# catniplab/vjf

Hardware: AMD Instinct MI355X
Metric: trial-timesteps/sec (higher is better)
Workload: dtype f32

## Files before the change

### include/vjf_hip.h

```cpp
#ifndef VJF_HIP_H
#define VJF_HIP_H

#include <stdint.h>

#ifdef __cplusplus
extern "C" {
#endif

#define VJF_ABI_VERSION 1
#define VJF_MAX_HIDDEN 8

#define VJF_LIK_GAUSSIAN 0
#define VJF_LIK_POISSON 1

#define VJF_FLAG_SGD 1u
#define VJF_FLAG_UPDATE 2u
#define VJF_FLAG_WARM_UP 4u
#define VJF_FLAG_EXACT_NONFINITE 8u

#define VJF_STATUS_NONFINITE_RECON 1u
#define VJF_STATUS_NONFINITE_DYN 2u
#define VJF_STATUS_NONFINITE_ENT 4u
#define VJF_STATUS_RLS_FAILED 8u
#define VJF_STATUS_WAIT_RESIDENT 0x100u
// ... 40 lines not shown
    VJF_SC_FREEZE_DEC = 6,
    VJF_SC_STATUS = 7,
    VJF_SC_TRI_CLEAN = 8,
    VJF_SC_SHRINK = 9,
    VJF_N_SCALARS = 16
};

typedef struct vjf_config {
    int32_t ydim, xdim, udim, n_rbf;
    int32_t n_hidden;
    int32_t hidden[VJF_MAX_HIDDEN];
    int32_t likelihood;
    int32_t max_batch;
    int32_t device;
} vjf_config;

#define VJF_ACT_TANH 0
#define VJF_ACT_RELU 1
#define VJF_ACT_LEAKY_RELU 2
#define VJF_ACT_ELU 3
#define VJF_ACT_SOFTPLUS 4
#define VJF_ACT_SIGMOID 5
#define VJF_ACT_HARDTANH 6
typedef struct vjf_activation { int32_t kind; float p0, p1; } vjf_activation;

typedef struct vjf_ctx vjf_ctx;

int vjf_abi_version(void);
const char* vjf_last_error(void);

int vjf_state_size(const vjf_config* cfg, int64_t* n_floats);
int vjf_state_layout(const vjf_config* cfg, int64_t* offsets, int64_t* sizes);
int vjf_workspace_size(const vjf_config* cfg, int64_t* bytes);

int vjf_ctx_create(const vjf_config* cfg, float* state, void* workspace, int64_t workspace_bytes,
                   void* stream, vjf_ctx** out);
int vjf_ctx_destroy(vjf_ctx* ctx);
int vjf_set_activation(vjf_ctx* ctx, const vjf_activation* act);
int vjf_set_stream(vjf_ctx* ctx, void* stream);
int vjf_get_status(vjf_ctx* ctx, uint32_t* status);

int vjf_set_overlap(vjf_ctx* ctx, int enable);

int vjf_route(vjf_ctx* ctx, uint32_t flags);

int vjf_comm_unique_id(void* ids256);
int vjf_comm_init(vjf_ctx* ctx, const void* ids256, int32_t rank, int32_t world);
int vjf_set_collectives(vjf_ctx* ctx, int32_t per_step);
int vjf_comm_ranks(vjf_ctx* ctx, int32_t* ranks2);

int vjf_debug_stamps(vjf_ctx* ctx, int enable, uint64_t* out32);

int vjf_filter_step(vjf_ctx* ctx, int32_t B, const float* y, const float* u, const float* mu_s,
                    const float* lv_s, const float* eps_s, const float* eps_t, float* mu_t, float* lv_t,
                    float* loss4, uint32_t flags);

int vjf_filter_local(vjf_ctx* ctx, int32_t B, const float* y, const float* u, const float* mu_s,
                     const float* lv_s, const float* eps_s, const float* eps_t, float* mu_t, float* lv_t,
                     uint32_t flags);
int vjf_reduce_buffer(vjf_ctx* ctx, float** ptr, int64_t* n_floats);
int vjf_filter_global(vjf_ctx* ctx, int32_t B_total, float* loss4, uint32_t flags);

int vjf_filter_seq(vjf_ctx* ctx, int32_t T, int32_t B, const float* y, const float* u, const float* eps,
                   const float* mu0, const float* lv0, float* mu, float* lv, float* loss, uint32_t flags);

int vjf_rbf_forward(const float* x, const float* centroid, const float* logwidth, float* out,
// ... 77 lines not shown
```

### vjf_amd/_native.py

```python
import ctypes as C
import os

HERE = os.path.dirname(os.path.abspath(__file__))
_variant = os.environ.get("VJF_LIB", "")
LIB_PATH = os.path.join(HERE, f"libvjf_hip_{_variant}.so" if _variant.isalnum() else "libvjf_hip.so")

ABI_VERSION = 1
MAX_HIDDEN = 8
LIK_GAUSSIAN, LIK_POISSON = 0, 1
FLAG_SGD, FLAG_UPDATE, FLAG_WARM_UP, FLAG_EXACT_NONFINITE = 1, 2, 4, 8
STATUS_NONFINITE_RECON, STATUS_NONFINITE_DYN, STATUS_NONFINITE_ENT, STATUS_RLS_FAILED = 1, 2, 4, 8
STATUS_NOT_RESIDENT, STATUS_WAIT_MASK = 0x20000, 0x3ff00

SLOT_PRIOR_MEAN, SLOT_PRIOR_LOGVAR, SLOT_LIK_LOGVAR, SLOT_TR_LOGVAR, SLOT_CENTROID, SLOT_LOGWIDTH = range(6)
SLOT_REC_W0, SLOT_REC_B0 = 6, 7
SLOT_MEAN_W, SLOT_LV_W, SLOT_LV_B, SLOT_DEC_W, SLOT_DEC_B = 22, 23, 24, 25, 26
SLOT_W_MEAN, SLOT_W_CHOL, SLOT_W_PREC, SLOT_W_PCHOL, SLOT_SCALARS = 27, 28, 29, 30, 31
N_SLOTS = 32
SC_N_LIK, SC_N_TR, SC_LR_LIK, SC_LR_DEC, SC_LR_TR, SC_LR_REC, SC_FREEZE_DEC, SC_STATUS, SC_TRI_CLEAN, SC_SHRINK = range(10)
N_SCALARS = 16


ACT_TANH, ACT_RELU, ACT_LEAKY_RELU, ACT_ELU, ACT_SOFTPLUS, ACT_SIGMOID, ACT_HARDTANH = range(7)


class VjfActivation(C.Structure):
    _fields_ = [("kind", C.c_int32), ("p0", C.c_float), ("p1", C.c_float)]


class VjfError(RuntimeError):
    """A C-ABI call returned an error code."""


class VjfConfig(C.Structure):
    _fields_ = [("ydim", C.c_int32), ("xdim", C.c_int32), ("udim", C.c_int32), ("n_rbf", C.c_int32),
                ("n_hidden", C.c_int32), ("hidden", C.c_int32 * MAX_HIDDEN), ("likelihood", C.c_int32),
                ("max_batch", C.c_int32), ("device", C.c_int32)]


_P = C.c_void_p
_I = C.c_int32
_U = C.c_uint32
_F = C.c_float

SIGNATURES = {
    "vjf_abi_version": [],
    "vjf_state_size": [C.POINTER(VjfConfig), C.POINTER(C.c_int64)],
    "vjf_state_layout": [C.POINTER(VjfConfig), C.POINTER(C.c_int64), C.POINTER(C.c_int64)],
    "vjf_workspace_size": [C.POINTER(VjfConfig), C.POINTER(C.c_int64)],
    "vjf_ctx_create": [C.POINTER(VjfConfig), _P, _P, C.c_int64, _P, C.POINTER(_P)],
    "vjf_ctx_destroy": [_P],
    "vjf_set_activation": [_P, C.POINTER(VjfActivation)],
    "vjf_set_stream": [_P, _P],
    "vjf_get_status": [_P, C.POINTER(_U)],
    "vjf_set_overlap": [_P, _I],
    "vjf_route": [_P, _U],
    "vjf_comm_unique_id": [_P],
    "vjf_comm_init": [_P, _P, _I, _I],
    "vjf_comm_ranks": [_P, C.POINTER(_I)],
    "vjf_set_collectives": [_P, _I],
    "vjf_debug_stamps": [_P, _I, C.POINTER(C.c_uint64)],
    "vjf_filter_step": [_P, _I, _P, _P, _P, _P, _P, _P, _P, _P, _P, _U],
    "vjf_filter_local": [_P, _I, _P, _P, _P, _P, _P, _P, _P, _P, _U],
    "vjf_reduce_buffer": [_P, C.POINTER(_P), C.POINTER(C.c_int64)],
    "vjf_filter_global": [_P, _I, _P, _U],
    "vjf_filter_seq": [_P, _I, _I, _P, _P, _P, _P, _P, _P, _P, _P, _U],
    "vjf_rbf_forward": [_P, _P, _P, _P, _I, _I, _I, _P],
    "vjf_blr_predict": [_P, _P, _P, _P, _P, _P, _P, _I, _I, _I, _I, _P],
    "vjf_blr_sample": [_P, _P, _P, _P, _P, _P, _P, _P, _I, _I, _I, _I, _P],
    "vjf_forecast_scratch_size": [_I, _I, _I, C.POINTER(C.c_int64)],
    "vjf_forecast_seq": [_P, _P, _P, _P, _P, _P, _P, _P, _P, _P, _P, _I, _I, _I, _I, _I, _P],
    "vjf_forecast_ens_scratch_size": [_I, _I, _I, _I, _I, C.POINTER(C.c_int64)],
    "vjf_forecast_ens_chunks": [_I, _I, _I, _I, _I, C.POINTER(_I), C.POINTER(_I)],
    "vjf_forecast_ens": [_P, C.c_int64] + [_P] * 16 + [_I] * 7 + [_P],
    "vjf_tangent_plan": [_I, _I, _I, _I, C.POINTER(_I), C.POINTER(C.c_int64)],
    "vjf_tangent_rollout": [_P] * 10 + [_I] * 8 + [_P],
    "vjf_fixed_points_plan": [_I, _I, _I, C.POINTER(C.c_int64)],
    "vjf_fixed_points": [_P] * 10 + [_I] * 5 + [_F, _F, _P],
    "vjf_smooth_plan": [_I, _I, _I, C.POINTER(C.c_int64)],
    "vjf_smooth": [_P] * 12 + [_I] * 5 + [_F, _P],
    "vjf_smooth_sample_plan": [_I, _I, _I, _I, C.POINTER(_I), C.POINTER(C.c_int64)],
    "vjf_smooth_sample": [_P] * 9 + [_I] * 6 + [_F, _P],
# ... 84 lines not shown
```

### vjf_amd/csrc/vjf_abi.hip

```cpp
#include <hip/hip_runtime.h>
#include <hip/hip_ext.h>

#include <dlfcn.h>

#include <cstdarg>
#include <cstdio>
#include <cstdlib>
#include <cstring>
#include <ctime>
#include <atomic>
#include <mutex>
#include <new>
#include <string>
#include <type_traits>
#include <vector>

#include "../../include/vjf_hip.h"
#include "vjf_chol_blocks.h"
#include "vjf_chol_kernel.h"
#include "vjf_gram_kernel.h"
#include "vjf_handoff.h"
#include "vjf_mega_kernel.h"
#include "vjf_ops_kernels.h"
#include "vjf_plan.h"
// ... 31 lines not shown
#else
#define VJF_CHAOS_REFRESH(c) ((void)0)
#endif

extern "C" {

int vjf_abi_version(void) { return VJF_ABI_VERSION; }
const char* vjf_last_error(void) { return g_err.c_str(); }

int vjf_state_size(const vjf_config* cfg, int64_t* n_floats) {
    VjfPlan P;
    if (int rc = plan_for("vjf_state_size", cfg, &P)) return rc;
    if (!n_floats) return fail(-1, "vjf_state_size: null output");
    *n_floats = P.n_state;
    return 0;
}

int vjf_state_layout(const vjf_config* cfg, int64_t* offsets, int64_t* sizes) {
    VjfPlan P;
    if (int rc = plan_for("vjf_state_layout", cfg, &P)) return rc;
    if (!offsets || !sizes) return fail(-1, "vjf_state_layout: null output");
    for (int s = 0; s < VJF_N_SLOTS; ++s) { offsets[s] = P.off[s]; sizes[s] = P.size[s]; }
    return 0;
}

int vjf_workspace_size(const vjf_config* cfg, int64_t* bytes) {
    VjfPlan P;
    if (int rc = plan_for("vjf_workspace_size", cfg, &P)) return rc;
    if (!bytes) return fail(-1, "vjf_workspace_size: null output");
    if (cfg->max_batch < 1) return fail(-7, "vjf_workspace_size: max_batch must be >= 1");
    std::vector<VjfJob> jobs;
    build_jobs(P, jobs);
    *bytes = (int64_t)carve_ws(P, cfg->max_batch, (int)jobs.size()).total;
    return 0;
}

int vjf_ctx_create(const vjf_config* cfg, float* state, void* workspace, int64_t workspace_bytes, void* stream,
                   vjf_ctx** out) {
    if (!cfg || !state || !workspace || !out) return fail(-1, "vjf_ctx_create: null argument");
    VjfPlan P;
    if (int rc = plan_for("vjf_ctx_create", cfg, &P)) return rc;
    if (cfg->max_batch < 1) return fail(-7, "vjf_ctx_create: max_batch must be >= 1");
    std::vector<VjfJob> jobs;
    build_jobs(P, jobs);
    if ((int)jobs.size() > VJF_MAX_JOBS) return fail(-8, "vjf_ctx_create: %zu Gram tiles exceed the limit", jobs.size());
    Carve cv = carve_ws(P, cfg->max_batch, (int)jobs.size());
    if ((int64_t)cv.total > workspace_bytes)
        return fail(-9, "vjf_ctx_create: workspace too small (%lld < %zu bytes)", (long long)workspace_bytes, cv.total);
    const size_t lds_k2 = vjf_serial_lds_floats(P) * 4;
    const bool fast_chol = vjf_chol_lds_ok(P);
    if (!fast_chol && lds_k2 > kMaxLds - 1024 && P.n <= 32 * VJF_CHOL_MAXBLK)
        return fail(-11, "vjf_ctx_create: n_rbf=%d too large for the single-workgroup RLS kernel", P.n);
    VJF_HIP(hipSetDevice(cfg->device));
    vjf_ctx* c = new (std::nothrow) vjf_ctx();
    if (!c) return fail(-12, "vjf_ctx_create: out of host memory");
    c->cfg = *cfg; c->plan = P; c->state = state; c->ws = (char*)workspace; c->ws_bytes = workspace_bytes;
    c->stream = (hipStream_t)stream; c->cv = cv; c->njobs = (int)jobs.size();
    c->lds_k2 = lds_k2;
    c->fast_chol = fast_chol;
    c->lds_post = vjf_post_lds_bytes(P);
    c->post_kernels = fast_chol && P.dz <= 16 && c->lds_post <= kMaxLds - 1024;
    c->lds_chol = fast_chol ? kMaxLds - 256 : vjf_chol_lds_bytes(P);
    if (c->post_kernels) c->lds_post = kMaxLds - 256;
    c->lds_k1m = vjf_trial_mfma_lds_floats(P) * 4;
    c->mfma_trial = c->lds_k1m <= kMaxLds - 1024;
    for (const VjfJob& j : jobs) c->n_ejobs += j.kind == 0;
    { const char* ha = getenv("VJF_HANDOFF_ACQUIRE"); c->handoff_acquire = ha && atoi(ha) != 0; }
    c->mega_ok = c->mega_plan = mega_plan_ok(P);
    VJF_HIP(hipDeviceGetAttribute(&c->ncu, hipDeviceAttributeMultiprocessorCount, cfg->device));
    if (const char* ce = getenv("VJF_COLLECTIVES")) { if (atoi(ce) == 1) c->collectives = 1; }
    hipError_t e = hipMemcpyAsync(c->jobs(), jobs.data(), jobs.size() * sizeof(VjfJob), hipMemcpyHostToDevice, c->stream);
    if (e == hipSuccess) e = hipMemsetAsync(c->red(), 0, (size_t)P.red_len * 4, c->stream);
    if (e == hipSuccess) e = hipMemsetAsync(c->red_rls(0), 0, (size_t)P.red_len * 4, c->stream);
    if (e == hipSuccess) e = hipMemsetAsync(c->red_rls(1), 0, (size_t)P.red_len * 4, c->stream);
    if (e == hipSuccess) e = hipMemsetAsync(c->flag_words(), 0, 256, c->stream);
    SlabTables tb;
    if (c->mega_ok) {
        const VjfMegaTrialLds Lo = vjf_mega_trial_lds(P, (int)(kMegaLds / 4) - 8);
        tb = slab_tables(P, Lo, vjf_mega_slab_layout(P));
        if (e == hipSuccess) e = hipMemcpyAsync(c->mg_pidx(), tb.pidx.data(), tb.pidx.size() * 4, hipMemcpyHostToDevice, c->stream);
        if (e == hipSuccess) e = hipMemcpyAsync(c->mg_cidx(), tb.cidx.data(), tb.cidx.size() * 4, hipMemcpyHostToDevice, c->stream);
        if (e == hipSuccess) e = hipMemcpyAsync(c->mg_grp(), tb.grp.data(), tb.grp.size() * 4, hipMemcpyHostToDevice, c->stream);
        if (e == hipSuccess) e = hipMemsetAsync(c->mg_img(), 0, (size_t)Lo.th_len * 4, c->stream);
        if (e == hipSuccess) e = hipMemsetAsync(c->mega_counters(0), 0, (size_t)2 * MG_C_WORDS * 4, c->stream);
    }
    if (e == hipSuccess) e = hipStreamSynchronize(c->stream);
    if (e != hipSuccess) { delete c; return fail(-100, "vjf_ctx_create: %s", hipGetErrorString(e)); }
    allow_lds(vjf_serial_kernel, c->lds_k2);
    allow_lds(vjf_rls_post_kernel, c->lds_post);
    allow_lds(vjf_prepg_kernel, vjf_prepg_lds_bytes(P));
    if (c->mfma_trial) allow_lds(vjf_trial_mfma_kernel<>, c->lds_k1m);
    allow_lds(chol_kernels(P.dz).chol, c->lds_chol);
    if (P.dz <= 16) allow_lds(chol_kernels(P.dz).pair, c->lds_chol);
    mega_residency(c);
    if (DevShared* d = dev_shared(cfg->device)) {
        std::lock_guard<std::mutex> lk(d->mu);
        if (!d->mirror_h) {
            unsigned* h = nullptr; unsigned* dp = nullptr;
            if (hipHostMalloc((void**)&h, VJF_MIRROR_WORDS * sizeof(unsigned), hipHostMallocMapped | hipHostMallocCoherent) == hipSuccess &&
                hipHostGetDevicePointer((void**)&dp, h, 0) == hipSuccess) {
                memset(h, 0, VJF_MIRROR_WORDS * sizeof(unsigned));
                d->mirror_h = h; d->mirror_d = dp;
            }
            (void)hipGetLastError();
        }
        count_mega(c, d);
    }
    *out = c;
    return 0;
}

int vjf_ctx_destroy(vjf_ctx* ctx) {
    if (!ctx) return 0;
    if (DevShared* d = dev_shared(ctx->cfg.device)) {
        std::lock_guard<std::mutex> lk(d->mu);
// ... 592 lines not shown
```

### vjf_amd/csrc/vjf_host_ctx.h

```cpp
#pragma once

namespace {

thread_local std::string g_err;

int fail(int code, const char* fmt, ...) {
    char buf[512];
    va_list ap;
    va_start(ap, fmt);
    vsnprintf(buf, sizeof buf, fmt, ap);
    va_end(ap);
    g_err = buf;
    return code;
}

#define VJF_HIP(call)                                                                            \
    do {                                                                                         \
        hipError_t e_ = (call);                                                                  \
        if (e_ != hipSuccess) return fail(-100, "%s failed: %s (%s:%d)", #call, hipGetErrorString(e_), __FILE__, __LINE__); \
    } while (0)

#define VJF_LAUNCH(kernel, grid, block, lds, st, stop, ...)                                             \
    do {                                                                                               \
        if (stop) hipExtLaunchKernelGGL(kernel, grid, block, (uint32_t)(lds), st, nullptr, stop, 0, __VA_ARGS__); \
// ... 216 lines not shown
struct Carve {
    size_t pscr; size_t mg_mom, mg_xt, mg_early, mg_late, mg_gslab, mg_cnt, mg_stamps, mg_pidx, mg_cidx, mg_grp, mg_img, mg_pmsave; size_t E, E2, ACT, DEL, partial, partial2, slabs, red, red2, red3, tbig, wide, work, jobs, aux, post, lscr, flags, resid, total;
};

Carve carve_ws(const VjfPlan& P, int max_batch, int njobs) {
    Carve c{};
    size_t o = 0;
    auto take = [&](size_t bytes) { size_t at = o; o = (o + bytes + 255) / 256 * 256; return at; };
    c.E = take((size_t)max_batch * P.ldE * 4);
    c.E2 = take((size_t)max_batch * P.ldE * 4);
    c.ACT = take((size_t)max_batch * P.ldA * 4);
    c.DEL = take((size_t)max_batch * P.ldD * 4);
    c.partial = take(((size_t)max_batch / 4 + 2) * RS_N * 4);
    c.partial2 = take(((size_t)max_batch / 4 + 2) * RS_N * 4);
    c.slabs = take((size_t)njobs * split_for(max_batch) * 1024 * 4);
    c.red = take((size_t)P.red_len * 4);
    c.red2 = take((size_t)P.red_len * 4);
    c.red3 = take((size_t)P.red_len * 4);
    c.tbig = take(P.n > 32 * VJF_CHOL_MAXBLK ? (size_t)((P.n + 31) / 32) * 1024 * 4 * 3 : 16);
    c.wide = take(vjf_trial_mfma_lds_floats(P) * 4 > kMaxLds - 1024 ? (size_t)max_batch * (P.dxu + P.dz + 1 + P.dy + P.n) * 4 + 1024 : 16);
    c.work = take(vjf_serial_work_floats(P) * 4 + 10 * 256);
    c.post = take((size_t)((P.n + 31) / 32) * 1024 * 4 + VJF_RESID_BLOCKS * 8 + 64);
    c.flags = take(256);
    c.lscr = take((size_t)P.n * P.n * 4);
    c.pscr = take((size_t)(VJF_CHOL_MAXBLK * (VJF_CHOL_MAXBLK + 1) / 2) * 1024 * 4);
    if (mega_plan_ok(P)) {
        const int nbl = (P.n + 31) / 32;
        const size_t slab_len = (size_t)vjf_mega_slab_layout(P).len;
        c.mg_early = take((size_t)2 * kMegaMaxTrialWg * ((size_t)((P.n + 3) & ~3) * 16 + 8) * 4);
        c.mg_late = take((size_t)kMegaMaxTrialWg * (slab_len + 8 * VJF_MG_RING) * 4);
        c.mg_gslab = take((size_t)kMegaMaxGramWg * (nbl * (nbl + 1) / 2) * 1024 * 4);
        c.mg_cnt = take((size_t)2 * MG_C_WORDS * 4);
        c.mg_stamps = take((32 * 32 + kMegaMaxTrialWg * 8) * 8);
        c.mg_pidx = take(slab_len * 4); c.mg_cidx = take(slab_len * 4); c.mg_grp = take(slab_len);
        c.mg_img = take((size_t)vjf_mega_trial_lds(P, (int)(kMegaLds / 4) - 8).th_len * 4 + 64);
        c.mg_pmsave = take((size_t)max_batch * (P.dz + 1) * 4);
        c.mg_xt = take((size_t)P.n * P.n * 4);
        {
            int nt = (max_batch + VJF_MG_TR - 1) / VJF_MG_TR;
            if (nt > VJF_MG_TAG_TILES) nt = VJF_MG_TAG_TILES;
            c.mg_mom = take((size_t)nt * 2 * (2 * P.dz + 1) * VJF_MG_TR * 4);
        }
    }
    c.jobs = take((size_t)njobs * sizeof(VjfJob));
    c.aux = take((size_t)P.aux_len * 4);
    c.resid = take(P.n > 32 * VJF_CHOL_MAXBLK ? (size_t)max_batch * P.dz * 4 : 16);
    c.total = o;
    return c;
}

template <class K>
void allow_lds(K kernel, size_t bytes) {
    (void)hipFuncSetAttribute(reinterpret_cast<const void*>(kernel), hipFuncAttributeMaxDynamicSharedMemorySize, (int)bytes);
    (void)hipGetLastError();
}

}

struct vjf_ctx {
    vjf_config cfg{};
    VjfPlan plan{};
    float* state = nullptr;
    char* ws = nullptr;
    int64_t ws_bytes = 0;
    hipStream_t stream = nullptr;
    Carve cv{};
    int njobs = 0;
// ... 13 lines not shown
    bool mega_ok = false;
    bool mega_plan = false;
    VjfAct act{VJF_ACT_TANH, 0.f, 0.f};
    bool ran = false;
    int ncu = 0;
    int mega_wg_per_cu = 0;
    int lite_wg_per_cu = 0;
    unsigned mega_launches = 0;
    hipStream_t stream2 = nullptr, stream3 = nullptr;
    hipEvent_t ev_s = nullptr, ev_c = nullptr;
    hipEvent_t ev_f[2] = {}, ev_r[2] = {}, ev_b[2] = {}, ev_g[2] = {};
    unsigned epoch = 0;
    unsigned k1_count = 0;
    unsigned post_count = 0;
    unsigned fwd_count = 0;
    unsigned stats_count = 0;
    unsigned start_count = 0;
    bool mega_counted = false;
    bool on_mega = false;
    void* comm_a = nullptr; void* comm_b = nullptr;
    int world = 1;
    int collectives = 2;
    int fake_world = 1;

    template <class T> T* at(size_t off) const { return reinterpret_cast<T*>(ws + off); }
#define VJF_WS_REGION(T, name) T* name() const { return at<T>(cv.name); }
    VJF_WS_REGION(float, ACT) VJF_WS_REGION(float, DEL) VJF_WS_REGION(float, slabs) VJF_WS_REGION(float, tbig) VJF_WS_REGION(float, wide)
    VJF_WS_REGION(float, work) VJF_WS_REGION(float, aux) VJF_WS_REGION(float, lscr) VJF_WS_REGION(float, pscr) VJF_WS_REGION(float, resid)
    VJF_WS_REGION(float, red)
    VJF_WS_REGION(VjfJob, jobs)
    VJF_WS_REGION(float, mg_mom) VJF_WS_REGION(float, mg_xt) VJF_WS_REGION(float, mg_early) VJF_WS_REGION(float, mg_late) VJF_WS_REGION(float, mg_gslab)
    VJF_WS_REGION(float, mg_img) VJF_WS_REGION(float, mg_pmsave) VJF_WS_REGION(int, mg_pidx) VJF_WS_REGION(int, mg_cidx) VJF_WS_REGION(int, mg_grp)
#undef VJF_WS_REGION
    float* E(int gen = 0) const { return at<float>(gen ? cv.E2 : cv.E); }
    float* partial(int gen = 0) const { return at<float>(gen ? cv.partial2 : cv.partial); }
    float* red_rls(int gen) const { return at<float>(gen ? cv.red3 : cv.red2); }
    float* status_word() const { return state + plan.off[VJF_SLOT_SCALARS] + VJF_SC_STATUS; }
    unsigned* flag_words() const { return at<unsigned>(cv.flags); }
    size_t dinv_bytes() const { return (size_t)((plan.n + 31) / 32) * 1024 * 4; }
    float* dinv() const { return at<float>(cv.post); }
    double* resid_partial() const { return at<double>(cv.post + dinv_bytes()); }
    int* ok_flag() const { return at<int>(cv.post + dinv_bytes() + VJF_RESID_BLOCKS * 8); }
    unsigned long long* step_stamps() const { return at<unsigned long long>(cv.work + vjf_serial_work_floats(plan) * 4); }
    unsigned long long* mega_stamps() const { return at<unsigned long long>(cv.mg_stamps); }
    unsigned* mega_counters(unsigned launch) const { return at<unsigned>(cv.mg_cnt) + (size_t)(launch & 1u) * MG_C_WORDS; }
};

namespace {
template <class KT, class KA, class F>
auto with_act_kernel(const VjfAct& act, KT tanh_kernel, KA act_kernel, F&& f) {
    if (act.kind == VJF_ACT_TANH) return f(tanh_kernel);
    return f(act_kernel, act);
}
template <class F> auto with_trial_kernel(const VjfAct& a, F&& f) { return with_act_kernel(a, vjf_trial_mfma_kernel<>, vjf_trial_mfma_kernel<VjfAct>, f); }
template <class F> auto with_mega_kernel(const VjfAct& a, F&& f) { return with_act_kernel(a, vjf_mega_kernel, vjf_mega_act_kernel, f); }
template <class F> auto with_lite_kernel(const VjfAct& a, F&& f) { return with_act_kernel(a, vjf_mega_lite_kernel, vjf_mega_lite_act_kernel, f); }

struct CholKernels { void (*chol)(VjfPlan, VjfCholArgs); void (*pair)(VjfPlan, VjfCholArgs, VjfPostArgs); };
CholKernels chol_kernels(int dz) {
    static const decltype(CholKernels::chol) chol[5] = {vjf_chol_lds_kernel<4>, vjf_chol_lds_kernel<8>, vjf_chol_lds_kernel<12>,
                                                        vjf_chol_lds_kernel<16>, vjf_chol_lds_kernel<32>};
    static const decltype(CholKernels::pair) pair[5] = {vjf_rls_pair_kernel<4>, vjf_rls_pair_kernel<8>, vjf_rls_pair_kernel<12>,
                                                        vjf_rls_pair_kernel<16>, nullptr};
    const int dzp = vjf_chol_dzp(dz), i = dzp <= 16 ? dzp / 4 - 1 : 4;
    return CholKernels{chol[i], pair[i]};
}
// ... 119 lines not shown
```

### vjf_amd/csrc/vjf_mega_common.h

```cpp
#pragma once
#include <hip/hip_runtime.h>
#include "vjf_chol_kernel.h"
#include "vjf_rls_operands.h"
#include "vjf_handoff.h"
#include "vjf_plan.h"
#include "vjf_post_kernel.h"
#include "vjf_trial_mfma_kernel.h"
#include "vjf_act.h"

#define VJF_MG_THREADS 512
#define VJF_MG_WAVES 8
#define VJF_MG_TR 32
#define VJF_MG_LD 33
#define VJF_MG_GROWS 96
#define VJF_MG_MAXQ 4
#define VJF_MG_RING 32
#define VJF_MG_TAG_TILES 512
#define RS_RESID 5

#ifndef MG_C_SPREAD
#define MG_C_SPREAD 1
#endif
enum {
    MG_C_FWD = 16 * MG_C_SPREAD,
// ... 435 lines not shown
    do {                                                                                    \
        if (A.stamps && tid == 0 && t == A.T - 1 && !replay) {                              \
            unsigned long long t_;                                                          \
            asm volatile("s_memrealtime %0\n\ts_waitcnt lgkmcnt(0)" : "=s"(t_)::"memory");  \
            A.stamps[1024 + (size_t)wg * 8 + (i)] = t_;                                     \
        }                                                                                   \
    } while (0)

__device__ __forceinline__ void mg_grad_tile(const float* D, int M, int m0, const float* Bact, int Kin, int j0, const float* s_one,
                                             const float* s_zero, float* blk, int ldm, int rows, bool first, int lane) {
    constexpr int LD = VJF_MG_LD;
    const int i = lane & 15, kk = lane >> 4;
    const float* arow = ((m0 + i) < M ? D + (size_t)(m0 + i) * LD : s_zero) + kk;
    const int jj = j0 + i;
    const float* brow = (jj < Kin ? Bact + (size_t)jj * LD : (jj == Kin ? s_one : s_zero)) + kk;
    float a[8], b[8];
#pragma unroll
    for (int s = 0; s < 8; ++s) { a[s] = arow[4 * s]; b[s] = brow[4 * s]; }
    vjf_f32x4 acc = {0.f, 0.f, 0.f, 0.f}, acc1 = {0.f, 0.f, 0.f, 0.f};
#pragma unroll
    for (int s = 0; s < 8; s += 2) {
        acc = __builtin_amdgcn_mfma_f32_16x16x4f32(a[s], b[s], acc, 0, 0, 0);
        acc1 = __builtin_amdgcn_mfma_f32_16x16x4f32(a[s + 1], b[s + 1], acc1, 0, 0, 0);
    }
    acc += acc1;
    const int mq = m0 + 4 * (lane >> 4), j = j0 + (lane & 15);
    if (j < rows && mq < ldm) {
        float* p = blk + (size_t)j * ldm + mq;
        if (!first) { acc[0] += vjf_ld_sc1(p); acc[1] += vjf_ld_sc1(p + 1); acc[2] += vjf_ld_sc1(p + 2); acc[3] += vjf_ld_sc1(p + 3); }
        vjf_st4_wt(p, acc[0], acc[1], acc[2], acc[3]);
    }
}

typedef __attribute__((address_space(3))) const float mg_lds_cf;
typedef __attribute__((address_space(1))) const float mg_glb_cf;
__device__ __forceinline__ void mg_sum_losses(const VjfMegaArgs& A, int t, float* s_sc, int tid, float Bf, int dz, bool want_resid) {
    const int ring = 8 * (t % VJF_MG_RING);
    if (tid < 32 * 5) {
        const int sc = tid >> 5, l = tid & 31, slot = sc < RS_SDX2 ? sc : RS_RESID;
        double d = 0.0;
        if (sc < RS_SDX2 || want_resid)
            for (int w = l; w < A.n_trial; w += 32) d += (double)vjf_ld_sc1(A.slab_late + (size_t)w * A.late_len + A.slab_len + ring + slot);
        d = vjf_sum32(d);
        if (l == 0) s_sc[slot] = slot == RS_RESID ? (float)(d / ((double)Bf * (double)dz)) : (float)d;
    }
    __syncthreads();
}

#define MG_PHASE()                                                        \
    do {                                                                  \
        tid = tid0;                                                       \
        asm volatile("" : "+v"(tid));                                     \
        lane = tid & 63;                                                  \
        wave = __builtin_amdgcn_readfirstlane(tid >> 6);                  \
    } while (0)

template <int NG, int LD>
__device__ __forceinline__ void mg_varN(float (&v2)[NG], __amdgpu_buffer_rsrc_t rx, int n, int j0A, int KA, int j0B, int KB, mg_lds_cf* Xs, int lane,
                                        const bool upper = true) {
    if (j0A < 0) return;
    const int i = lane & 15, kk = lane >> 4;
    const bool rvA = (j0A + i) < n, rvB = j0B >= 0 && (j0B + i) < n;
    const int offA = (rvA ? j0A + i : 0) * n + 4 * kk, offB = (rvB ? j0B + i : 0) * n + 4 * kk;
    mg_lds_cf* xp = Xs + i;
    const int ntA = (KA + 15) >> 4, ntB = j0B >= 0 ? (KB + 15) >> 4 : 0;
    const int SA = (ntA + 3) >> 2, SB = (ntB + 3) >> 2, S = SA + SB;
    vjf_f32x4 acc[NG];
#pragma unroll
// ... 85 lines not shown
```

### vjf_amd/csrc/vjf_mega_trial.h

```cpp
#pragma once
#include "vjf_mega_common.h"

template <bool RLS, bool ACT = false>
__device__ __forceinline__ void vjf_mega_trial(const VjfPlan& P, const VjfMegaArgs& A, float* smem, const int wg, const VjfAct act = VjfAct{}) {
    constexpr int LD = VJF_MG_LD, NW = VJF_MG_WAVES, NT = VJF_MG_THREADS, TR = VJF_MG_TR;
    constexpr bool VSPLIT = RLS && !ACT;
    const int tid0 = threadIdx.x;
    const int dz = P.dz, dy = P.dy, du = P.du, n = P.n, din = P.din, dxu = P.dxu;
    const float* S = A.state;
    float* SCW = A.state + P.off[VJF_SLOT_SCALARS];
    const bool do_sgd = RLS || (A.flags & VJF_FLAG_SGD) != 0u, do_upd = RLS || (A.flags & VJF_FLAG_UPDATE) != 0u;
    const bool warm = !RLS && (A.flags & VJF_FLAG_WARM_UP) != 0u;
    constexpr bool mode_rls = RLS;
    const bool gated = RLS || do_sgd || do_upd;
    const bool want_resid = !RLS && do_upd && warm;
    const bool use_mom = !RLS && A.n_mom > 0;
    const unsigned m_dy = mg_magic(dy), m_dz = mg_magic(dz), m_du = mg_magic(du > 0 ? du : 1);
    const VjfMegaTrialLds Lo = vjf_mega_trial_lds<false>(P, A.lds_floats);
    const bool tl = Lo.theta != 0;
    float* s_cen = smem + Lo.cen; float* s_iw = smem + Lo.iw;
    float* s_in = smem + Lo.in; float* s_xu = smem + Lo.xu; float* s_phi = smem + Lo.phi; float* s_act = smem + Lo.act;
    float* s_dd = smem + Lo.dd;
    float* s_mu = smem + Lo.mu; float* s_lv = smem + Lo.lv; float* s_xt = smem + Lo.xt; float* s_e2 = smem + Lo.e2; float* s_pm = smem + Lo.pm;
    float* s_dmu = smem + Lo.dmu; float* s_dlv = smem + Lo.dlv; float* s_dx = smem + Lo.dx;
    float* s_py = smem + Lo.py; float* s_dpy = smem + Lo.dpy;
    float* s_one = smem + Lo.one; float* s_zero = smem + Lo.zero;
    float* s_sc = smem + Lo.sc; float* s_red = smem + Lo.red; float* s_plv = smem + Lo.plv; float* s_wg = smem + Lo.wg;
    const bool compact = dy >= P.hmax;
    float* s_d0 = compact ? s_py : s_dd;
    float* s_d1 = compact ? s_dd : s_dd + P.hmax * LD;
    float* s_part = smem + Lo.part;
    constexpr int part_rows = VJF_MG_WAVES * 16;
    int mean_nsl = 1;
    __shared__ unsigned s_try[2];
    unsigned* cnt = A.cnt;
    const unsigned npost = (unsigned)(A.n_rls - 1);
    float* late = A.slab_late + (size_t)wg * A.late_len;
    const int ldn = (n + 3) & ~3;
    const size_t sy = (size_t)A.B * dy, su = (size_t)A.B * du, sz = (size_t)A.B * dz;
// ... 526 lines not shown
                float ldyn = 0.f, ent = 0.f, rsd = 0.f;
                {
                    const float p = expf(-0.5f * sig), e = expf(-sig), plv = s_plv[b];
                    for (int j = s; j < dz; j += LPT) {
                        if (want_resid) { const float r = s_dx[j * LD + b] - s_dmu[j * LD + b]; rsd = fmaf(r, r, rsd); }
                        const VjfDynSeed sd = vjf_dyn_term(s_pm[j * LD + b], s_mu[j * LD + b], s_lv[j * LD + b], plv, sig, p, e, !warm && m_d, m_h, ldyn, ent);
                        s_dmu[j * LD + b] = ok ? sd.dmu : 0.f;
                        s_dlv[j * LD + b] = ok ? sd.dlv : 0.f;
                    }
                }
                ldyn = group_sum<LPT>(ldyn);
                ent = group_sum<LPT>(ent);
                if (want_resid) rsd = group_sum<LPT>(rsd);
                if (s == 0) {
                    s_sc[b * RS_N + RS_RESID] = ok ? rsd : 0.f;
                    s_sc[b * RS_N + RS_LRECON] = ok ? lrec : 0.f;
                    s_sc[b * RS_N + RS_LDYN] = ok ? ldyn : 0.f;
                    s_sc[b * RS_N + RS_ENT] = ok ? ent : 0.f;
                    s_sc[b * RS_N + RS_SSEY] = ok ? ssey : 0.f;
                }
            }
            __syncthreads(); MG_PHASE();
            if (first) VJF_MG_STAMP(31);
#ifdef VJF_EXPERIMENT_SLOW_TRIAL
            { const unsigned long long t0_ = wall_clock64(); while (wall_clock64() - t0_ < VJF_EXPERIMENT_SLOW_TRIAL) __builtin_amdgcn_s_sleep(1); }
#endif
            if ((tid < RS_SDX2 || (tid == RS_RESID && want_resid)) && !replay) {
                float v = 0.f;
                for (int bb = 0; bb < TR; ++bb) v += s_sc[bb * RS_N + tid];
                s_wg[tid] += v;
            }
            if (do_sgd) {
            int gbase = 0;
            auto grad_tensor = [&](const float* D, int M, const float* Bact, int Kin, int blkid) {
                int b_off, b_ldm, b_rows;
                mg_slab_block(P, blkid, b_off, b_ldm, b_rows);
                const int ntm = (M + 15) >> 4, ntj = (Kin + 1 + 15) >> 4;
                const unsigned mj = mg_magic(ntj);
                for (int q = (wave - gbase) & (NW - 1); q < ntm * ntj; q += NW) {
                    const int tm = mg_div(q, mj), tj = q - tm * ntj;
                    mg_grad_tile(D, M, tm * 16, Bact, Kin, tj * 16, s_one, s_zero, late + b_off, b_ldm, b_rows, first, lane);
                }
                gbase += ntm * ntj;
            };
            {
                const float* C = S + P.off[VJF_SLOT_DEC_W];
                const int mt = (dz + 15) >> 4;
                float* s_kp = compact ? s_py : s_dd;
                const int rows_av = compact ? dy : Lo.nd * P.hmax;
                const int nslb = min(NW / mt, rows_av / (16 * mt));
                if (nslb >= 2) {
                    if (wave < mt * nslb) {
                        const int tt = wave / nslb, sl = wave - tt * nslb;
                        const int per = (((dy + 3) >> 2) + nslb - 1) / nslb * 4;
                        vjf_f32x4 acc0 = {0.f, 0.f, 0.f, 0.f}, acc1 = {0.f, 0.f, 0.f, 0.f};
                        if (tl) mg_mma2_lds<true>(acc0, acc1, smem + Lo.th_dec, Lo.th_ldd, dz, tt * 16, s_dpy, sl * per, min(dy, (sl + 1) * per), lane);
                        else mg_mma2(acc0, acc1, C, dz, dz, tt * 16, s_dpy, sl * per, min(dy, (sl + 1) * per), lane);
                        float* pr = s_kp + (size_t)((sl * mt + tt) * 16 + 4 * (lane >> 4)) * LD + (lane & 15);
#pragma unroll
                        for (int r = 0; r < 4; ++r) { pr[r * LD] = acc0[r]; pr[r * LD + 16] = acc1[r]; }
                    }
                    __syncthreads(); MG_PHASE();
                    for (int e = tid; e < TR * dz; e += NT) {
                        const int j = e >> 5, b = e & 31;
                        float a = 0.f;
                        for (int sl = 0; sl < nslb; ++sl) a += s_kp[(size_t)((sl * mt + (j >> 4)) * 16 + (j & 15)) * LD + b];
// ... 45 lines not shown
                                mg_mma2(acc0, acc1, Wm, hL, hL, tt * 16, s_dmu, 0, dz, lane);
                                mg_mma2(acc0, acc1, Wl, hL, hL, tt * 16, s_dlv, 0, dz, lane);
                            }
                        } else if (tl) {
                            mg_mma2_lds<true>(acc0, acc1, smem + d_w, d_ldw, hp, tt * 16, src, 0, P.h[l], lane);
                        } else {
                            mg_mma2(acc0, acc1, S + P.off[VJF_SLOT_REC_W0 + 2 * l], hp, hp, tt * 16, src, 0, P.h[l], lane);
                        }
#pragma unroll
                        for (int r = 0; r < 4; ++r) {
                            const int k = tt * 16 + 4 * (lane >> 4) + r, b = lane & 15;
                            if (k < hp) {
                                const float h0 = hprev[k * LD + b], h1 = hprev[k * LD + 16 + b];
                                if (ACT) {
                                    dst[k * LD + b] = acc0[r] * vjf_act_dh(act, h0);
                                    dst[k * LD + 16 + b] = acc1[r] * vjf_act_dh(act, h1);
                                } else {
                                    dst[k * LD + b] = acc0[r] * (1.f - h0 * h0);
                                    dst[k * LD + 16 + b] = acc1[r] * (1.f - h1 * h1);
                                }
                            }
                        }
                    }
                };
                auto layer_grads = [&](int l, const float* da) {
                    int aoff = 0;
                    for (int q = 0; q < l - 1; ++q) aoff += P.h[q];
                    grad_tensor(da, P.h[l], l > 0 ? s_act + aoff * LD : s_in, l > 0 ? P.h[l - 1] : din, 3 + (P.L - 1 - l));
                };
                delta(P.L, nullptr, s_d0);
                __syncthreads(); MG_PHASE();
                if (P.L >= 2) { delta(P.L - 1, s_d0, s_d1); __syncthreads(); MG_PHASE(); }
                if (first) VJF_MG_STAMP(19);
                grad_tensor(s_dpy, dy, s_xt, dz, 0);
                grad_tensor(s_dmu, dz, hact, hL, 1);
                grad_tensor(s_dlv, dz, hact, hL, 2);
                layer_grads(P.L - 1, s_d0);
                if (P.L >= 2) layer_grads(P.L - 2, s_d1);
                float* cur = s_d1; float* nxt = s_d0;
                for (int l = P.L - 3; l >= 0; --l) {
                    __syncthreads(); MG_PHASE();
                    delta(l + 1, cur, nxt);
                    __syncthreads(); MG_PHASE();
                    layer_grads(l, nxt);
                    float* tmp = cur; cur = nxt; nxt = tmp;
                }
            }
            }
            if (first) { VJF_MG_STAMP(8); VJF_MG_STAMPW(4); }
            if (last) {
                __syncthreads(); MG_PHASE();
                if ((tid < RS_SDX2 || (tid == RS_RESID && want_resid)) && !replay) vjf_st_wt(late + A.slab_len + 8 * (tc % VJF_MG_RING) + tid, s_wg[tid]);
                if (gated) vjf_wg_signal_wt(cnt + (replay ? MG_C_REDO_B : MG_C_BWD), tid);
                else {
                    vjf_chaos(tid, cnt + MG_C_ARR, 2);
                    asm volatile("s_waitcnt vmcnt(0)" ::: "memory");
                    __syncthreads();
                    if (tid == 0) s_try[0] = __hip_atomic_fetch_add(cnt + MG_C_ARR + (tc % VJF_MG_RING), 1u, __ATOMIC_RELAXED, __HIP_MEMORY_SCOPE_AGENT) + 1u == (unsigned)A.n_trial ? 1u : 0u;
                    __syncthreads(); MG_PHASE();
                    if (s_try[0]) {
                        float* s_tot = s_sc;
                        mg_sum_losses(A, tc, s_tot, tid, (float)A.B, dz, false);
                        if (tid == 0) {
                            const VjfLossVerdict v = vjf_loss_verdict(s_tot[RS_LRECON], s_tot[RS_LDYN], s_tot[RS_ENT], 1.0f / (float)A.B, warm);
                            if (A.loss) vjf_put_loss4(A.loss + 4 * (size_t)tc, v);
                            if (v.status()) vjf_status_or(SCW + VJF_SC_STATUS, v.status());
                            __hip_atomic_store(cnt + MG_C_ARR + (tc % VJF_MG_RING), 0u, __ATOMIC_RELAXED, __HIP_MEMORY_SCOPE_AGENT);
                            asm volatile("s_waitcnt vmcnt(0)" ::: "memory");
                            __hip_atomic_fetch_add(cnt + MG_C_SGD, 1u, __ATOMIC_RELAXED, __HIP_MEMORY_SCOPE_AGENT);
                        }
                        __syncthreads(); MG_PHASE();
                    }
                }
                VJF_MG_STAMP(9);
                VJF_MG_STAMPX(29, 30);
                VJF_MG_STAMPW(5);
            }
// ... 18 lines not shown
```

Measured before the change: 83.07 million.

## Precompute gradient tile table on host and walk it in the mega kernel

Adds a host-built table of gradient MFMA tiles (LDS offsets, bounds, slab destinations) copied into workspace. On the RLS-without-activation path, the kernel walks this flat table per wave with scalar constant loads instead of recomputing per-tensor tile decomposition with magic division. This is meant to remove index arithmetic and per-tensor loop overhead and to balance tiles across waves. It costs extra workspace and a table upload at context creation. A look-ahead variant exists but is not the one used.

```diff
diff --git a/include/vjf_hip.h b/include/vjf_hip.h
--- a/include/vjf_hip.h
+++ b/include/vjf_hip.h
@@ -96,6 +96,7 @@
 int vjf_state_size(const vjf_config* cfg, int64_t* n_floats);
 int vjf_state_layout(const vjf_config* cfg, int64_t* offsets, int64_t* sizes);
 int vjf_workspace_size(const vjf_config* cfg, int64_t* bytes);
+int vjf_mega_grad_tile_table(const vjf_config* cfg, int32_t* table, int32_t capacity, int32_t* n_words);
 
 int vjf_ctx_create(const vjf_config* cfg, float* state, void* workspace, int64_t workspace_bytes,
                    void* stream, vjf_ctx** out);
diff --git a/vjf_amd/_native.py b/vjf_amd/_native.py
--- a/vjf_amd/_native.py
+++ b/vjf_amd/_native.py
@@ -48,6 +48,7 @@
     "vjf_state_size": [C.POINTER(VjfConfig), C.POINTER(C.c_int64)],
     "vjf_state_layout": [C.POINTER(VjfConfig), C.POINTER(C.c_int64), C.POINTER(C.c_int64)],
     "vjf_workspace_size": [C.POINTER(VjfConfig), C.POINTER(C.c_int64)],
+    "vjf_mega_grad_tile_table": [C.POINTER(VjfConfig), C.POINTER(_I), _I, C.POINTER(_I)],
     "vjf_ctx_create": [C.POINTER(VjfConfig), _P, _P, C.c_int64, _P, C.POINTER(_P)],
     "vjf_ctx_destroy": [_P],
     "vjf_set_activation": [_P, C.POINTER(VjfActivation)],
diff --git a/vjf_amd/csrc/vjf_abi.hip b/vjf_amd/csrc/vjf_abi.hip
--- a/vjf_amd/csrc/vjf_abi.hip
+++ b/vjf_amd/csrc/vjf_abi.hip
@@ -87,6 +87,17 @@
     std::vector<VjfJob> jobs;
     build_jobs(P, jobs);
     *bytes = (int64_t)carve_ws(P, cfg->max_batch, (int)jobs.size()).total;
+    return 0;
+}
+
+int vjf_mega_grad_tile_table(const vjf_config* cfg, int32_t* table, int32_t capacity, int32_t* n_words) {
+    VjfPlan P;
+    if (int rc = plan_for("vjf_mega_grad_tile_table", cfg, &P)) return rc;
+    const int words = vjf_mega_grad_tiles(P, nullptr);
+    if (n_words) *n_words = words;
+    if (!table) return 0;
+    if (capacity < words) return fail(-7, "vjf_mega_grad_tile_table: capacity %d < %d words", (int)capacity, words);
+    vjf_mega_grad_tiles(P, table);
     return 0;
 }
 
@@ -130,12 +141,16 @@
     if (e == hipSuccess) e = hipMemsetAsync(c->red_rls(1), 0, (size_t)P.red_len * 4, c->stream);
     if (e == hipSuccess) e = hipMemsetAsync(c->flag_words(), 0, 256, c->stream);
     SlabTables tb;
+    std::vector<int> gtab;
     if (c->mega_ok) {
         const VjfMegaTrialLds Lo = vjf_mega_trial_lds(P, (int)(kMegaLds / 4) - 8);
         tb = slab_tables(P, Lo, vjf_mega_slab_layout(P));
         if (e == hipSuccess) e = hipMemcpyAsync(c->mg_pidx(), tb.pidx.data(), tb.pidx.size() * 4, hipMemcpyHostToDevice, c->stream);
         if (e == hipSuccess) e = hipMemcpyAsync(c->mg_cidx(), tb.cidx.data(), tb.cidx.size() * 4, hipMemcpyHostToDevice, c->stream);
         if (e == hipSuccess) e = hipMemcpyAsync(c->mg_grp(), tb.grp.data(), tb.grp.size() * 4, hipMemcpyHostToDevice, c->stream);
+        gtab.resize((size_t)vjf_mega_grad_tiles(P, nullptr));
+        vjf_mega_grad_tiles(P, gtab.data());
+        if (e == hipSuccess) e = hipMemcpyAsync(c->mg_gtab(), gtab.data(), gtab.size() * 4, hipMemcpyHostToDevice, c->stream);
         if (e == hipSuccess) e = hipMemsetAsync(c->mg_img(), 0, (size_t)Lo.th_len * 4, c->stream);
         if (e == hipSuccess) e = hipMemsetAsync(c->mega_counters(0), 0, (size_t)2 * MG_C_WORDS * 4, c->stream);
     }
diff --git a/vjf_amd/csrc/vjf_host_ctx.h b/vjf_amd/csrc/vjf_host_ctx.h
--- a/vjf_amd/csrc/vjf_host_ctx.h
+++ b/vjf_amd/csrc/vjf_host_ctx.h
@@ -272,7 +272,7 @@
         c.mg_gslab = take((size_t)kMegaMaxGramWg * (nbl * (nbl + 1) / 2) * 1024 * 4);
         c.mg_cnt = take((size_t)2 * MG_C_WORDS * 4);
         c.mg_stamps = take((32 * 32 + kMegaMaxTrialWg * 8) * 8);
-        c.mg_pidx = take(slab_len * 4); c.mg_cidx = take(slab_len * 4); c.mg_grp = take(slab_len);
+        c.mg_pidx = take(slab_len * 4); c.mg_cidx = take(slab_len * 4); c.mg_grp = take((size_t)(VJF_GT_AT((int)slab_len) + vjf_mega_grad_tiles(P, nullptr)) * 4);
         c.mg_img = take((size_t)vjf_mega_trial_lds(P, (int)(kMegaLds / 4) - 8).th_len * 4 + 64);
         c.mg_pmsave = take((size_t)max_batch * (P.dz + 1) * 4);
         c.mg_xt = take((size_t)P.n * P.n * 4);
@@ -352,6 +352,7 @@
     VJF_WS_REGION(float, mg_mom) VJF_WS_REGION(float, mg_xt) VJF_WS_REGION(float, mg_early) VJF_WS_REGION(float, mg_late) VJF_WS_REGION(float, mg_gslab)
     VJF_WS_REGION(float, mg_img) VJF_WS_REGION(float, mg_pmsave) VJF_WS_REGION(int, mg_pidx) VJF_WS_REGION(int, mg_cidx) VJF_WS_REGION(int, mg_grp)
 #undef VJF_WS_REGION
+    int* mg_gtab() const { return mg_grp() + VJF_GT_AT(vjf_mega_slab_layout(plan).len); }
     float* E(int gen = 0) const { return at<float>(gen ? cv.E2 : cv.E); }
     float* partial(int gen = 0) const { return at<float>(gen ? cv.partial2 : cv.partial); }
     float* red_rls(int gen) const { return at<float>(gen ? cv.red3 : cv.red2); }
diff --git a/vjf_amd/csrc/vjf_mega_common.h b/vjf_amd/csrc/vjf_mega_common.h
--- a/vjf_amd/csrc/vjf_mega_common.h
+++ b/vjf_amd/csrc/vjf_mega_common.h
@@ -491,8 +491,101 @@
     }
 }
 
+#define VJF_GT_HDR 16
+#define VJF_GT_ENT 8
+#define VJF_GT_AT(slab_len) ((((slab_len) >> 2) + 7) & ~7)
+static inline int vjf_mega_grad_tiles(const VjfPlan& P, int* tab) {
+    constexpr int LD = VJF_MG_LD;
+    const VjfMegaTrialLds Lo = vjf_mega_trial_lds(P);
+    const VjfMegaSlab SL = vjf_mega_slab_layout(P);
+    const bool compact = P.dy >= P.hmax;
+    const int d0 = compact ? Lo.py : Lo.dd, d1 = compact ? Lo.dd : Lo.dd + P.hmax * LD;
+    const int hL = P.h[P.L - 1];
+    int nt = 0, nseg = 0;
+    if (tab) for (int k = 0; k < VJF_GT_HDR; ++k) tab[k] = 0;
+    auto tensor = [&](int D, int M, int Bact, int Kin, int blk) {
+        const int ntm = (M + 15) >> 4, ntj = (Kin + 1 + 15) >> 4, ldm = SL.ldm[blk], rows = SL.rows[blk];
+        for (int tm = 0; tm < ntm; ++tm)
+            for (int tj = 0; tj < ntj; ++tj) {
+                const int m0 = 16 * tm, j0 = 16 * tj;
+                if (rows - j0 <= 0 || ldm - m0 <= 0) continue;
+                if (tab) {
+                    int* e = tab + VJF_GT_HDR + VJF_GT_ENT * nt;
+                    e[0] = D + m0 * LD; e[1] = M - m0; e[2] = Bact + j0 * LD; e[3] = Kin - j0;
+                    e[4] = SL.off[blk] + j0 * ldm + m0; e[5] = ldm; e[6] = rows - j0; e[7] = ldm - m0;
+                }
+                ++nt;
+            }
+    };
+    auto layer = [&](int l) {
+        int aoff = 0;
+        for (int q = 0; q < l - 1; ++q) aoff += P.h[q];
+        tensor(((P.L - 1 - l) & 1) ? d1 : d0, P.h[l], l > 0 ? Lo.act + aoff * LD : Lo.in, l > 0 ? P.h[l - 1] : P.din, 3 + (P.L - 1 - l));
+    };
+    auto close = [&]() { if (tab) tab[2 + nseg] = nt; ++nseg; };
+    tensor(Lo.dpy, P.dy, Lo.xt, P.dz, 0);
+    tensor(Lo.dmu, P.dz, Lo.act + (P.hsum - hL) * LD, hL, 1);
+    tensor(Lo.dlv, P.dz, Lo.act + (P.hsum - hL) * LD, hL, 2);
+    layer(P.L - 1);
+    if (P.L >= 2) layer(P.L - 2);
+    close();
+    for (int l = P.L - 3; l >= 0; --l) { layer(l); close(); }
+    if (tab) { tab[0] = nt; tab[1] = nseg; }
+    return VJF_GT_HDR + VJF_GT_ENT * nt;
+}
+
+typedef __attribute__((address_space(4))) const int mg_cst_i;
+typedef int mg_i8 __attribute__((ext_vector_type(8)));
+typedef __attribute__((address_space(4))) const mg_i8 mg_cst_i8;
 typedef __attribute__((address_space(3))) const float mg_lds_cf;
 typedef __attribute__((address_space(1))) const float mg_glb_cf;
+
+template <bool LOOK>
+__device__ __forceinline__ void mg_grad_walk(const int* table, int& q, const int qend, const float* smem, const int one, const int zero,
+                                             float* late, const bool first, const int lane) {
+    constexpr int LD = VJF_MG_LD, NW = VJF_MG_WAVES;
+    mg_cst_i* tab = (mg_cst_i*)table + VJF_GT_HDR;
+    mg_lds_cf* lds = (mg_lds_cf*)smem;
+    const int i = lane & 15, kk = lane >> 4, row = i * LD + kk;
+    auto ent = [&](int qq) { return *(const mg_cst_i8*)(tab + VJF_GT_ENT * qq); };
+    auto rd = [&](const mg_i8 e, float (&a)[8], float (&b)[8]) {
+        const int ao = i < e[1] ? e[0] + row : zero + kk;
+        const int bo = i < e[3] ? e[2] + row : ((i == e[3] ? one : zero) + kk);
+#pragma unroll
+        for (int s = 0; s < 8; ++s) { a[s] = lds[ao + 4 * s]; b[s] = lds[bo + 4 * s]; }
+    };
+    auto fin = [&](const mg_i8 e, const float (&a)[8], const float (&b)[8]) {
+        vjf_f32x4 acc = {0.f, 0.f, 0.f, 0.f}, acc1 = {0.f, 0.f, 0.f, 0.f};
+#pragma unroll
+        for (int s = 0; s < 8; s += 2) {
+            acc = __builtin_amdgcn_mfma_f32_16x16x4f32(a[s], b[s], acc, 0, 0, 0);
+            acc1 = __builtin_amdgcn_mfma_f32_16x16x4f32(a[s + 1], b[s + 1], acc1, 0, 0, 0);
+        }
+        acc += acc1;
+        if (i < e[6] && 4 * kk < e[7]) {
+            float* p = late + e[4] + i * e[5] + 4 * kk;
+            if (!first) { acc[0] += vjf_ld_sc1(p); acc[1] += vjf_ld_sc1(p + 1); acc[2] += vjf_ld_sc1(p + 2); acc[3] += vjf_ld_sc1(p + 3); }
+            vjf_st4_wt(p, acc[0], acc[1], acc[2], acc[3]);
+        }
+    };
+    if (LOOK) {
+        float a0[8], b0[8], a1[8], b1[8];
+        mg_i8 e0 = {}, e1 = {};
+        if (q < qend) { e0 = ent(q); rd(e0, a0, b0); }
+        while (q < qend) {
+            if (q + NW < qend) { e1 = ent(q + NW); rd(e1, a1, b1); }
+            fin(e0, a0, b0);
+            q += NW;
+            if (q >= qend) break;
+            if (q + NW < qend) { e0 = ent(q + NW); rd(e0, a0, b0); }
+            fin(e1, a1, b1);
+            q += NW;
+        }
+    } else {
+        float a[8], b[8];
+        for (; q < qend; q += NW) { const mg_i8 e = ent(q); rd(e, a, b); fin(e, a, b); }
+    }
+}
 __device__ __forceinline__ void mg_sum_losses(const VjfMegaArgs& A, int t, float* s_sc, int tid, float Bf, int dz, bool want_resid) {
     const int ring = 8 * (t % VJF_MG_RING);
     if (tid < 32 * 5) {
diff --git a/vjf_amd/csrc/vjf_mega_trial.h b/vjf_amd/csrc/vjf_mega_trial.h
--- a/vjf_amd/csrc/vjf_mega_trial.h
+++ b/vjf_amd/csrc/vjf_mega_trial.h
@@ -5,6 +5,7 @@
 __device__ __forceinline__ void vjf_mega_trial(const VjfPlan& P, const VjfMegaArgs& A, float* smem, const int wg, const VjfAct act = VjfAct{}) {
     constexpr int LD = VJF_MG_LD, NW = VJF_MG_WAVES, NT = VJF_MG_THREADS, TR = VJF_MG_TR;
     constexpr bool VSPLIT = RLS && !ACT;
+    constexpr bool GTAB = RLS && !ACT;
     const int tid0 = threadIdx.x;
     const int dz = P.dz, dy = P.dy, du = P.du, n = P.n, din = P.din, dxu = P.dxu;
     const float* S = A.state;
@@ -597,6 +598,11 @@
             }
             if (do_sgd) {
             int gbase = 0;
+            int gq = wave;
+            auto grad_walk = [&](int seg) {
+                const int* gtab = A.sl_grp + VJF_GT_AT(A.slab_len);
+                mg_grad_walk<false>(gtab, gq, ((mg_cst_i*)gtab)[2 + seg], smem, Lo.one, Lo.zero, late, first, lane);
+            };
             auto grad_tensor = [&](const float* D, int M, const float* Bact, int Kin, int blkid) {
                 int b_off, b_ldm, b_rows;
                 mg_slab_block(P, blkid, b_off, b_ldm, b_rows);
@@ -708,17 +714,21 @@
                 __syncthreads(); MG_PHASE();
                 if (P.L >= 2) { delta(P.L - 1, s_d0, s_d1); __syncthreads(); MG_PHASE(); }
                 if (first) VJF_MG_STAMP(19);
-                grad_tensor(s_dpy, dy, s_xt, dz, 0);
-                grad_tensor(s_dmu, dz, hact, hL, 1);
-                grad_tensor(s_dlv, dz, hact, hL, 2);
-                layer_grads(P.L - 1, s_d0);
-                if (P.L >= 2) layer_grads(P.L - 2, s_d1);
+                if constexpr (GTAB) grad_walk(0);
+                else {
+                    grad_tensor(s_dpy, dy, s_xt, dz, 0);
+                    grad_tensor(s_dmu, dz, hact, hL, 1);
+                    grad_tensor(s_dlv, dz, hact, hL, 2);
+                    layer_grads(P.L - 1, s_d0);
+                    if (P.L >= 2) layer_grads(P.L - 2, s_d1);
+                }
                 float* cur = s_d1; float* nxt = s_d0;
                 for (int l = P.L - 3; l >= 0; --l) {
                     __syncthreads(); MG_PHASE();
                     delta(l + 1, cur, nxt);
                     __syncthreads(); MG_PHASE();
-                    layer_grads(l, nxt);
+                    if constexpr (GTAB) grad_walk(P.L - 2 - l);
+                    else layer_grads(l, nxt);
                     float* tmp = cur; cur = nxt; nxt = tmp;
                 }
             }
```

Measured after the change: 84.85 million (median of 6 runs). +2.1%, better.
